# tjysdsg/speech-recognition

Measured on AMD Instinct MI355X. Metric: frame-state loglik/s + utterances/s Viterbi decode, higher is better.
Workload: dtype f64; 1 GPU; configs[1]: 10-digit HMM, 5 states/digit, 8-mix GMM, 39-dim, 10000 utterances/GPU (999364 frames on rank 0), isolated-word decode; states=50, mixtures=8, dim=39, parallelism=utterance-sharded x1, batches_in_flight=2, process_group=single

## Files before the change

include/gmmhmm.h:

```cpp
#ifndef GMMHMM_H
#define GMMHMM_H

#include <stdint.h>

#ifdef __cplusplus
extern "C" {
#endif

typedef enum {
    GH_OK = 0,
    GH_ERR_INVALID = -1,
    GH_ERR_HIP = -2,
    GH_ERR_NOMEM = -3,
    GH_ERR_NODEVICE = -4,
    GH_ERR_SELF_POINTER = -5,
    GH_ERR_UNSUPPORTED = -6,
    GH_ERR_COMM = -7
} gh_status;

typedef enum { GH_F32 = 0, GH_F64 = 1 } gh_dtype;

typedef struct gh_ctx gh_ctx;
typedef struct gh_gmm gh_gmm;
typedef struct gh_batch gh_batch;
// ... 56 lines not shown
                 int64_t* end , int32_t* n_segments , uint8_t* open ,
                 int64_t* frames_done , const int64_t* frame_off , uint8_t* out_is_speech,
                 double* out_level, double* out_background, double* out_energy);
int gh_batch_create_from_pcm_endpointed(gh_ctx* ctx, gh_dtype dtype, int mode, int sample_fmt, int sample_rate,
                                        double frame_size, double frame_stride, double low_freq, double high_freq, int64_t U,
                                        const void* samples, const int64_t* sample_off, const gh_endpoint_params* prm,
                                        int start_boundary, int max_segments, int64_t* start, int64_t* end,
                                        int32_t* n_segments, uint8_t* open, int64_t* utt_frame_off, int64_t* n_utt,
                                        gh_batch** out);

int gh_loglik(gh_ctx* ctx, const gh_gmm* g, gh_batch* b, void* out_host );
int gh_loglik_subset(gh_ctx* ctx, const gh_gmm* g, gh_batch* b, const int32_t* state_lo ,
                     const int32_t* state_hi );
int gh_loglik_sets(gh_ctx* ctx, const gh_gmm* g, gh_batch* b, const int64_t* range_off ,
                   const int32_t* state_lo, const int32_t* state_hi);
void* gh_loglik_dev_ptr(gh_batch* b);
int gh_loglik_fetch(gh_ctx* ctx, const gh_batch* b, void* out_host );
int gh_component_loglik(gh_ctx* ctx, const gh_gmm* g, int state, int64_t N,
                        const double* x_host , double* out_host );
int gh_distance_matrix(gh_ctx* ctx, int64_t N, int K, int D, const double* x_host ,
                       const double* y_host , const double* var_host, int var_rows,
                       double* out_host );

int gh_lattices_create(gh_ctx* ctx, int L,
                       const int64_t* row_off , const int32_t* row_state,
                       const int64_t* arc_off , const int32_t* arc_to,
                       const int32_t* arc_from, const double* arc_cost,
                       const int64_t* start_off , const int32_t* start_rows,
                       const int64_t* end_off , const int32_t* end_rows,
                       gh_lattices** out);
// ... 134 lines not shown
```

speech-recognition_amd/csrc/gh_ctx.hip:

```cpp
#include "gh_internal.h"
#include "gh_host.h"

static thread_local std::string g_err;

void gh_set_error(const char* fmt, ...) {
    char buf[1024];
    va_list ap;
    va_start(ap, fmt);
    vsnprintf(buf, sizeof buf, fmt, ap);
    va_end(ap);
    g_err = buf;
}

extern "C" const char* gh_last_error(void) { return g_err.c_str(); }
extern "C" int gh_version(void) { return 1; }

extern "C" int gh_ctx_create(int device, gh_ctx** out) {
    GH_REQUIRE(out, "gh_ctx_create: out is NULL");
    *out = nullptr;
    int n = 0;
    hipError_t e = hipGetDeviceCount(&n);
    if (e != hipSuccess || n <= 0) {
        gh_set_error("gh_ctx_create: no HIP device (%s)", hipGetErrorString(e));
        return GH_ERR_NODEVICE;
// ... 5 lines not shown
    c->scratch = nullptr;
    c->scratch_bytes = 0;
    c->pinned = nullptr;
    c->pinned_bytes = 0;
    c->last_chunks = 0;
    c->compat = 1;
    if (const char* e = getenv("GMMHMM_COMPAT")) c->compat = strstr(e, "underflow") ? 1 : atoi(e);
    if (const char* e = getenv("GMMHMM_LSE")) if (!strcmp(e, "f32exp")) c->compat |= 2;
    hipDeviceProp_t prop;
    GH_HIP(hipGetDeviceProperties(&prop, device));
    c->n_cu = prop.multiProcessorCount;
    GH_HIP(hipStreamCreateWithFlags(&c->stream, hipStreamNonBlocking));
    GH_HIP(hipMalloc((void**)&c->d_flag, sizeof(int)));
    GH_HIP(hipMemset(c->d_flag, 0, sizeof(int)));
    {
        double t[384];
        for (int j = 0; j < 128; ++j) {
            t[j] = (double)exp2l((long double)j / 128.0L);
            const double inv = (double)(1.0L / (0.5L + ((long double)j + 0.5L) / 256.0L));
            t[128 + j] = inv;
            t[256 + j] = (double)(-logl((long double)inv) * (long double)GH_LSE_SCALE64);
        }
        GH_HIP(hipMalloc((void**)&c->d_fp64_tables, sizeof t));
        GH_HIP(hipMemcpy(c->d_fp64_tables, t, sizeof t, hipMemcpyHostToDevice));
    }
    *out = c;
    return GH_OK;
}

extern "C" void gh_ctx_destroy(gh_ctx* c) {
    if (!c) return;
    hipSetDevice(c->device);
    hipStreamSynchronize(c->stream);
    if (c->scratch) hipFree(c->scratch);
    if (c->pinned) hipHostFree(c->pinned);
    if (c->fit_arena) hipFree(c->fit_arena);
    if (c->fit_pin) hipHostFree(c->fit_pin);
// ... 115 lines not shown
```

speech-recognition_amd/csrc/gh_internal.h:

```cpp
#pragma once
#include <hip/hip_runtime.h>
#include <stdint.h>
#include <stdarg.h>
#include <stdio.h>
#include <string>
#include <vector>
#include "../../include/gmmhmm.h"

void gh_set_error(const char* fmt, ...);

#define GH_HIP(call)                                                                     \
    do {                                                                                 \
        hipError_t e_ = (call);                                                          \
        if (e_ != hipSuccess) {                                                          \
            gh_set_error("%s:%d %s -> %s", __FILE__, __LINE__, #call, hipGetErrorString(e_)); \
            return (e_ == hipErrorOutOfMemory) ? GH_ERR_NOMEM : GH_ERR_HIP;              \
        }                                                                                \
    } while (0)

#define GH_REQUIRE(cond, ...)                 \
    do {                                      \
        if (!(cond)) {                        \
            gh_set_error(__VA_ARGS__);        \
            return GH_ERR_INVALID;            \
// ... 21 lines not shown
    int last_fused = 0;
    int last_chunks;
    size_t budget_cache = 0;
    int budget_age = 0;
    void* fit_arena = nullptr;
    size_t fit_arena_bytes = 0;
    void* fit_pin = nullptr;
    void* fit_act = nullptr;
    size_t fit_act_bytes = 0;
};

int gh_scratch(gh_ctx* ctx, size_t bytes, void** out);
size_t gh_scratch_budget(gh_ctx* ctx, bool fresh = false);
int gh_pinned(gh_ctx* ctx, size_t bytes, void** out);

struct gh_gmm {
    gh_ctx* ctx;
    void* d_arena;
    int S, M, D, KP;
    std::vector<double> hA, hB, hC;
    bool host_stale = false;
    double *dA64, *dB64, *dC64;
    float *dA32, *dB32, *dC32;
    float* dCen32;
    double *dMean, *dIvar, *dLogc;
    int* dAnyPos = nullptr;
    int any_pos_host = -1;
    int M_pad, n_tiles;
    double *dApk64, *dCpk64;
    float *dApk32, *dCpk32;
// ... 189 lines not shown
```

speech-recognition_amd/csrc/gh_loglik_mfma.hip:

```cpp
#include "gh_internal.h"
#include "gh_wave.h"

namespace {

typedef double v4d __attribute__((ext_vector_type(4)));
typedef float v4f __attribute__((ext_vector_type(4)));

struct gh_loglik_blk { int64_t n0; int32_t nrows, t0, t1, pad; };

template <typename T> struct Acc;
template <> struct Acc<double> {
    typedef v4d type;
    static __device__ __forceinline__ v4d mfma(double a, double b, v4d c) {
        return __builtin_amdgcn_mfma_f64_16x16x4f64(a, b, c, 0, 0, 0);
    }
};
template <> struct Acc<float> {
    typedef v4f type;
    static __device__ __forceinline__ v4f mfma(float a, float b, v4f c) {
        return __builtin_amdgcn_mfma_f32_16x16x4f32(a, b, c, 0, 0, 0);
    }
};

struct Fp64Tables {
    double exp2[128];
    double inv[128];
    double nlog[128];
};

template <typename T> struct Dom;
template <> struct Dom<double> {
    static constexpr double inv_k = 1.0 / GH_LSE_SCALE64, off = GH_LSE_OFF64, off_test = GH_LSE_OFF64 * 0.1;
};
template <> struct Dom<float> {
    static constexpr float inv_k = (float)(1.0 / GH_LSE_SCALE32), off = GH_LSE_OFF32, off_test = GH_LSE_OFF32 * 0.1f;
};

struct LseK {
    double e3 = 2.6466421444330968834e-08;
    double l4 = -46.166241308446829036, l3 = 61.554988411262438714;
    double l2 = -92.332482616893658071, l1 = 184.66496523378731614;
    __device__ __forceinline__ void pin() {
        asm volatile("" : "+v"(e3), "+v"(l4), "+v"(l3), "+v"(l2), "+v"(l1));
    }
};

__device__ __forceinline__ double logs(double s, const double* __restrict__ tab, const LseK& k) {
    const double* __restrict__ inv = tab + 128;
    const double* __restrict__ nlog = tab + 256;
    const double m = __builtin_amdgcn_frexp_mant(s);
    const int e = __builtin_amdgcn_frexp_exp(s);
    const int j = (__double2hiint(m) >> 13) & 127;
    const double rho = fma(m, inv[j], -1.0);
    double p = fma(rho, 36.932993046757463228, k.l4);
    p = fma(p, rho, k.l3);
    p = fma(p, rho, k.l2);
    p = fma(p, rho, k.l1);
    return fma(p, rho, nlog[j]) + (double)(e << 7);
}
__device__ __forceinline__ float logs(float s, const double*, const LseK&) { return __builtin_amdgcn_logf(s); }

template <int W> __device__ __forceinline__ void swap_rows(unsigned v, unsigned& a, unsigned& b) {
    if (W == 16) {
        auto r = __builtin_amdgcn_permlane16_swap(v, v, false, false);
        a = r[0]; b = r[1];
    } else {
        auto r = __builtin_amdgcn_permlane32_swap(v, v, false, false);
        a = r[0]; b = r[1];
    }
}
template <int W> __device__ __forceinline__ void pair_of(float v, float& a, float& b) {
    unsigned x, y;
    swap_rows<W>(__float_as_uint(v), x, y);
    a = __uint_as_float(x); b = __uint_as_float(y);
}
// ... 11 lines not shown
}
__device__ __forceinline__ void pair_split(double v0, double v1, double& a, double& b) {
    auto lo = __builtin_amdgcn_permlane16_swap((unsigned)__double2loint(v0), (unsigned)__double2loint(v1), false, false);
    auto hi = __builtin_amdgcn_permlane16_swap((unsigned)__double2hiint(v0), (unsigned)__double2hiint(v1), false, false);
    a = __hiloint2double((int)hi[0], (int)lo[0]); b = __hiloint2double((int)hi[1], (int)lo[1]);
}
template <typename T> __device__ __forceinline__ T pair_sum_split(T v0, T v1) { T a, b; pair_split(v0, v1, a, b); return a + b; }
template <typename T> __device__ __forceinline__ T pair_max_split(T v0, T v1) { T a, b; pair_split(v0, v1, a, b); return vmax(a, b); }

template <typename T> __device__ __forceinline__ T nll_of(T mx, T sm, const double* tab, T inf_below, const LseK& k) {
    const T v = (mx + logs(sm, tab, k)) * -Dom<T>::inv_k;
    return (mx < inf_below) ? T(INFINITY) : v;
}

template <typename T, typename V> __device__ __forceinline__ T lane_max(const V& a) { return vmax(vmax(a[0], a[1]), vmax(a[2], a[3])); }
template <typename T, typename V> __device__ __forceinline__ T lane_terms(const V& a, T m, const double* tab, const LseK& k) {
    return (exp2s(a[0] - m, tab, k.e3) + exp2s(a[1] - m, tab, k.e3)) + (exp2s(a[2] - m, tab, k.e3) + exp2s(a[3] - m, tab, k.e3));
}
template <typename T, typename V>
__device__ __forceinline__ void tile_lse(const V& a, int width, T& mx, T& sm, const double* tab, const LseK& k) {
    T m = lane_max<T, V>(a);
    if (width >= 2) m = pair_max<T, 16>(m);
    if (width >= 4) m = pair_max<T, 32>(m);
    T e = lane_terms<T, V>(a, m, tab, k);
    if (width >= 2) e = pair_sum<T, 16>(e);
    if (width >= 4) e = pair_sum<T, 32>(e);
    mx = m;
    sm = e;
}

__device__ __forceinline__ float exp2s_fe(double y) { return __builtin_amdgcn_exp2f((float)y * 0.0078125f); }
template <int W> __device__ __forceinline__ float pair_sum_f(float v) { float a, b; pair_of<W>(v, a, b); return a + b; }
template <typename V>
__device__ __forceinline__ void tile_lse_fe(const V& a, int width, double& mx, float& sm) {
    double m = vmax(vmax(a[0], a[1]), vmax(a[2], a[3]));
    if (width >= 2) m = pair_max<double, 16>(m);
    if (width >= 4) m = pair_max<double, 32>(m);
    float e = (exp2s_fe(a[0] - m) + exp2s_fe(a[1] - m)) + (exp2s_fe(a[2] - m) + exp2s_fe(a[3] - m));
    if (width >= 2) e = pair_sum_f<16>(e);
// ... 1 lines not shown
    mx = m;
    sm = e;
}
__device__ __forceinline__ double nll_of_fe(double mx, float sm, double inf_below) {
    const double v = (mx + (double)(128.0f * __builtin_amdgcn_logf(sm))) * -Dom<double>::inv_k;
    return (mx < inf_below) ? (double)INFINITY : v;
}

template <typename T> using global_ptr = const T __attribute__((address_space(1)))*;
template <typename T> __device__ __forceinline__ global_ptr<T> uniform_ptr(const T* p) {
    uint32_t lo = (uint32_t)reinterpret_cast<uintptr_t>(p), hi = (uint32_t)(reinterpret_cast<uintptr_t>(p) >> 32);
    asm("" : "+s"(lo), "+s"(hi));
    return (global_ptr<T>)reinterpret_cast<const T*>(((uintptr_t)hi << 32) | lo);
}

template <typename T, typename V, int MP, bool FE = false>
__device__ __forceinline__ void tile_epilogue(const V& acc0, const V& acc1, int t, int f, int q, int S, int RS,
                                              int chunk_s0, int tiles_per_state, T* lds, T* dummy,
                                              const double* tab, T (&run_mx)[2], T (&run_sm)[2], T inf_below, const LseK& k) {
    T* orow0 = lds + f * RS - chunk_s0;
    T* orow1 = orow0 + 16 * RS;
    if (MP == 1) {
        const int s = 16 * t + 4 * q;
#pragma unroll
        for (int c = 0; c < 2; ++c) {
            const V& acc = c ? acc1 : acc0;
            T* orow = c ? orow1 : orow0;
#pragma unroll
            for (int r = 0; r < 4; ++r)
                *((s + r < S) ? orow + s + r : dummy) = (acc[r] < inf_below) ? T(INFINITY) : acc[r] * -Dom<T>::inv_k;
        }
    } else if (MP == 2) {
        const int s = 8 * t + 2 * q;
#pragma unroll
        for (int c = 0; c < 2; ++c) {
            const V& acc = c ? acc1 : acc0;
            T* orow = c ? orow1 : orow0;
#pragma unroll
            for (int h = 0; h < 2; ++h) {
                const T x0 = acc[2 * h], x1 = acc[2 * h + 1];
                const T m = vmax(x0, x1);
                const T e = exp2s(x0 - m, tab, k.e3) + exp2s(x1 - m, tab, k.e3);
                *((s + h < S) ? orow + s + h : dummy) = nll_of<T>(m, e, tab, inf_below, k);
            }
        }
#ifdef GH_MF_NOEPI
    } else if (MP <= 16) {
        const int s = (16 / MP) * t + q / (MP / 4);
        *(((q & (MP / 4 - 1)) == 0 && s < S) ? orow0 + s : dummy) = -((acc0[0] + acc0[1]) + (acc0[2] + acc0[3]));
        *(((q & (MP / 4 - 1)) == 0 && s < S) ? orow1 + s : dummy) = -((acc1[0] + acc1[1]) + (acc1[2] + acc1[3]));
#endif
    } else if (FE && MP == 4) {
        if constexpr (FE) {
            double mx; float sm;
            const int s = 4 * t + q;
            tile_lse_fe<V>(acc0, 1, mx, sm);
            *((s < S) ? orow0 + s : dummy) = nll_of_fe(mx, sm, inf_below);
            tile_lse_fe<V>(acc1, 1, mx, sm);
// ... 24 lines not shown
                run_sm[c] = (double)((d > 0.0) ? fmaf(smf, e, rs) : fmaf(rs, e, smf));
                run_mx[c] = (d > 0.0) ? run_mx[c] : mx;
            }
            const bool odd = q & 1;
            const double v = nll_of_fe(odd ? run_mx[1] : run_mx[0], (float)(odd ? run_sm[1] : run_sm[0]), inf_below);
            *((last && q < 2 && s < S) ? (odd ? orow1 : orow0) + s : dummy) = v;
#pragma unroll
            for (int c = 0; c < 2; ++c) {
                run_mx[c] = last ? Dom<T>::off : run_mx[c];
                run_sm[c] = last ? T(0) : run_sm[c];
            }
        }
    } else if (MP == 4) {
        T mx, sm;
        const int s = 4 * t + q;
        tile_lse<T, V>(acc0, 1, mx, sm, tab, k);
        *((s < S) ? orow0 + s : dummy) = nll_of<T>(mx, sm, tab, inf_below, k);
        tile_lse<T, V>(acc1, 1, mx, sm, tab, k);
        *((s < S) ? orow1 + s : dummy) = nll_of<T>(mx, sm, tab, inf_below, k);
    } else if (MP <= 16) {
        constexpr int width = MP / 4;
        T mxs = pair_max_split(lane_max<T, V>(acc0), lane_max<T, V>(acc1));
        if (width >= 4) mxs = pair_max<T, 32>(mxs);
        T mx0, mx1;
        pair_of<16>(mxs, mx0, mx1);
        T sm = pair_sum_split(lane_terms<T, V>(acc0, mx0, tab, k), lane_terms<T, V>(acc1, mx1, tab, k));
        if (width >= 4) sm = pair_sum<T, 32>(sm);
        const bool odd = q & 1;
        const int s = (16 / MP) * t + q / width;
        const T v = nll_of<T>(mxs, sm, tab, inf_below, k);
        *(((q & (width - 1)) < 2 && s < S) ? (odd ? orow1 : orow0) + s : dummy) = v;
    } else {
        const bool last = (t + 1) % tiles_per_state == 0;
        const int s = t / tiles_per_state;
#pragma unroll
        for (int c = 0; c < 2; ++c) {
            T mx, sm;
            tile_lse<T, V>(c ? acc1 : acc0, 4, mx, sm, tab, k);
            const T d = run_mx[c] - mx;
            const T e = exp2s((d > T(0)) ? -d : d, tab, k.e3);
            run_sm[c] = (d > T(0)) ? fma(sm, e, run_sm[c]) : fma(run_sm[c], e, sm);
            run_mx[c] = (d > T(0)) ? run_mx[c] : mx;
        }
        const bool odd = q & 1;
        const T v = nll_of<T>(odd ? run_mx[1] : run_mx[0], odd ? run_sm[1] : run_sm[0], tab, inf_below, k);
        *((last && q < 2 && s < S) ? (odd ? orow1 : orow0) + s : dummy) = v;
#pragma unroll
        for (int c = 0; c < 2; ++c) {
            run_mx[c] = last ? Dom<T>::off : run_mx[c];
            run_sm[c] = last ? T(0) : run_sm[c];
        }
    }
}

#ifndef GH_MF_SGB
#define GH_MF_SGB 0
#endif
template <typename T, int KS, int MP, bool MULTI, bool FE = false>
__global__ __launch_bounds__(64, (sizeof(T) == 4 ? 3 : 1)) void loglik_mfma_kernel(const T* __restrict__ X, int64_t N, int D,
                                                         const T* __restrict__ Apk, const T* __restrict__ Cpk,
                                                         int n_tiles, int S, int M_pad, int chunk_tiles,
                                                         const double* __restrict__ tables, int tab_off,
                                                         T* __restrict__ out, int bpw,
                                                         const gh_loglik_blk* __restrict__ blk_tab, int64_t n_blk,
                                                         const T* __restrict__ cen, T inf_below) {
    typedef typename Acc<T>::type V;
#ifndef GH_MF_RING32
#define GH_MF_RING32 2
#endif
#ifndef GH_MF_RING64
#define GH_MF_RING64 1
#endif
    constexpr int R = KS / (sizeof(T) == 4 ? GH_MF_RING32 : GH_MF_RING64);
    extern __shared__ __attribute__((aligned(16))) unsigned char smem_raw[];
    T* lds = reinterpret_cast<T*>(smem_raw);
    const int lane = threadIdx.x;
    const int f = lane & 15, q = lane >> 4;
    const int64_t n_blocks = (N + 31) / 32;
    int64_t n0 = (int64_t)blockIdx.x * (MULTI ? bpw : 1) * 32;
#ifdef GH_MF_TIMING
    long long tk[5], tw[2];
    tk[0] = clock64(); tw[0] = wall_clock64();
#endif
    int nrows = 0;
    const bool subset = MULTI && blk_tab != nullptr;
    const int64_t kb0 = (int64_t)blockIdx.x * (MULTI ? bpw : 1);
    int t_lo = subset ? blk_tab[kb0].t0 : 0, t_hi = n_tiles, nxt_t0 = 0;
    double* tab = reinterpret_cast<double*>(smem_raw + tab_off);
    if (sizeof(T) == 8 && MP != 1) {
        double tr[6];
#pragma unroll
        for (int it = 0; it < 6; ++it) tr[it] = tables[lane + 64 * it];
#pragma unroll
        for (int it = 0; it < 6; ++it) tab[lane + 64 * it] = tr[it];
    }
    auto stage_frames = [&]() {
        const int nelem = nrows * D;
        const T* src = X + n0 * D;
        T xr[KS];
#pragma unroll
        for (int it = 0; it < KS; ++it) {
            const int i = lane + 64 * it;
            xr[it] = (i < nelem) ? src[i] : T(0);
        }
#pragma unroll
        for (int it = 0; it < KS; ++it) {
            const int i = lane + 64 * it;
            if (i < nelem) lds[i] = xr[it];
        }
// ... 112 lines not shown
#ifdef GH_MF_PRIO
            __builtin_amdgcn_s_setprio(0);
#endif
            staged_n0 = n0;
        }
        chunk_s0 = (MP <= 16) ? t_lo * (16 / (MP <= 16 ? MP : 16)) : t_lo / tiles_per_state;
        if (subset) {
            const int s_end = (MP <= 16) ? t_hi * (16 / (MP <= 16 ? MP : 16)) : t_hi / tiles_per_state;
            subset_cnt = ((s_end < S) ? s_end : S) - chunk_s0;
        }
#ifdef GH_MF_TIMING
        tk[1] = clock64();
        tk[2] = tk[1];
#endif
        auto epi = [&](const V& e0, const V& e1, int t) {
            tile_epilogue<T, V, MP, FE>(e0, e1, t, f, q, S, RS, chunk_s0, tiles_per_state, lds, dummy, tab, run_mx, run_sm, inf_below, lse_k);
#pragma unroll
            for (int i = 0; i < (GH_MF_SGB ? 2 * KS : 0); ++i) {
                __builtin_amdgcn_sched_group_barrier(0x008, 1, 0);
                __builtin_amdgcn_sched_group_barrier(0x002, sizeof(T) == 8 ? 5 : 3, 0);
            }
            if (!subset && (t + 1) % chunk_tiles == 0 && t + 1 < n_tiles) flush();
        };
        V r0, r1;
        const int tb = MULTI ? t_lo : 0, te = MULTI ? t_hi : n_tiles;
        mfma_tile(tb, p0, p1, c_a, c_b);
        if (sizeof(T) == 8) {
            int t = tb + 1;
            for (; t + 1 < te; t += 2) {
                mfma_tile(t, r0, r1, c_b, c_a);
                epi(p0, p1, t - 1);
// ... 23 lines not shown
        tk[3] = clock64();
#endif
        flush();
#ifdef GH_MF_TIMING
        tk[4] = clock64(); tw[1] = wall_clock64();
        if (lane == 0 && S >= 8) {
            T* o = out + n0 * S;
            for (int i = 0; i < 5; ++i) o[i] = (T)(double)(tk[i] - tk[0]);
            o[5] = (T)(double)(tw[0] & 0xffffffffffll); o[6] = (T)(double)(tw[1] - tw[0]);
            o[7] = (T)(double)__builtin_amdgcn_s_getreg((4 << 0) | (0 << 6) | (31 << 11));
        }
#endif
    }
}

static void chunk_shape(const gh_gmm* g, int* chunk_tiles_out, int* SC_out) {
    const int M_pad = g->M_pad, n_tiles = g->n_tiles, S = g->S;
    int chunk_tiles;
    if (M_pad <= 16) {
        const int spt = 16 / M_pad;
        chunk_tiles = (S <= 64) ? n_tiles : std::max(1, 64 / spt);
    } else {
        const int tps = M_pad / 16;
        chunk_tiles = (S <= 64) ? n_tiles : 64 * tps;
    }
    *chunk_tiles_out = chunk_tiles;
    *SC_out = (M_pad <= 16) ? chunk_tiles * (16 / M_pad) : chunk_tiles / (M_pad / 16);
}

static int build_blk_table(const gh_gmm* g, const gh_batch* b, int SC, const int32_t* st_lo, const int32_t* st_hi,
                           const int64_t* rng_off, std::vector<gh_loglik_blk>& tabv, int* max_tiles_out,
                           const uint8_t* include = nullptr) {
    const int M_pad = g->M_pad, S = g->S;
    int max_tiles = 1;
    std::vector<std::pair<int, int>> runs;
    for (int64_t u = 0; u < b->U; ++u) {
        if (include && !include[u]) continue;
        runs.clear();
        const int64_t r0 = rng_off ? rng_off[u] : u, r1 = rng_off ? rng_off[u + 1] : u + 1;
        for (int64_t r = r0; r < r1; ++r) {
            const int lo = st_lo[r], hi = st_hi[r];
            if (lo < 0 || hi > S || lo >= hi) { gh_set_error("gh_loglik_subset: utterance %lld has state range [%d, %d)", (long long)u, lo, hi); return GH_ERR_INVALID; }
// ... 20 lines not shown
                tabv.push_back(gh_loglik_blk{f, (int32_t)std::min<int64_t>(32, b->offsets[u + 1] - f), tr.first, tr.second, 0});
    }
    *max_tiles_out = max_tiles;
    return GH_OK;
}

template <typename T>
int launch_mfma_t(gh_ctx* ctx, const gh_gmm* g, gh_batch* b, const T* Apk, const T* Cpk, const int32_t* st_lo,
                  const int32_t* st_hi, const T* cen, const int64_t* rng_off, const gh_loglik_plan* plan) {
    const int64_t N = b->N;
    if (N == 0) return GH_OK;
    const int KS = g->KP / 2;
    const int M_pad = g->M_pad, n_tiles = g->n_tiles, S = g->S;
    int chunk_tiles, SC;
    chunk_shape(g, &chunk_tiles, &SC);
    size_t lds = ((size_t)32 * std::max(std::min(SC, S), g->D) + 64) * sizeof(T);
    lds = (lds + 15) & ~size_t(15);
    const int tab_off = (int)lds;
    if (sizeof(T) == 8 && M_pad != 1) lds += 384 * sizeof(double);
    const double* tables = ctx->d_fp64_tables;
    const T inf_below = (ctx->compat & 1) ? (T)(-745.1332191019412 * (sizeof(T) == 8 ? GH_LSE_SCALE64 : GH_LSE_SCALE32)) : Dom<T>::off_test;
    gh_loglik_blk* d_blk = nullptr;
    int64_t n_blk = 0;
    int max_tiles = n_tiles;
    if (plan) {
        d_blk = static_cast<gh_loglik_blk*>(plan->d_blk);
        n_blk = plan->n_blk;
        max_tiles = plan->max_tiles;
        if (n_blk == 0) return GH_OK;
    } else if (st_lo) {
        std::vector<gh_loglik_blk> tabv;
        int rc = build_blk_table(g, b, SC, st_lo, st_hi, rng_off, tabv, &max_tiles);
        if (rc) return rc;
        n_blk = (int64_t)tabv.size();
// ... 3 lines not shown
        if (rc) return rc;
        d_blk = static_cast<gh_loglik_blk*>(base);
        GH_HIP(hipMemcpyAsync(d_blk, tabv.data(), tabv.size() * sizeof(gh_loglik_blk), hipMemcpyHostToDevice, ctx->stream));
        GH_HIP(hipStreamSynchronize(ctx->stream));
    }
    const bool subset = plan || st_lo;
    const int64_t n_blocks = subset ? n_blk : (N + 31) / 32;
    const int per_block = std::max(1, max_tiles * KS * 2);
    int bpw = (int)std::max<int64_t>(1, std::min<int64_t>(8, (512 + per_block - 1) / per_block));
    if (const char* e = getenv("GMMHMM_LOGLIK_BPW")) bpw = std::max(1, std::min(16, atoi(e)));
    if (subset) bpw = std::max(bpw, 2);
    const unsigned grid = (unsigned)((n_blocks + bpw - 1) / bpw);
    const T* X = static_cast<const T*>(b->feats);
    T* out = static_cast<T*>(b->nll);
    const bool fe = sizeof(T) == 8 && (ctx->compat & 2) && M_pad >= 4;
#define GH_MF_LAUNCH(ks, mp)                                                                                             \
    do {                                                                                                                 \
        if (fe && sizeof(T) == 8 && mp >= 4) {                                                                           \
            if (bpw > 1)                                                                                                 \
                hipLaunchKernelGGL((loglik_mfma_kernel<T, ks, mp, true, (sizeof(T) == 8 && mp >= 4)>), dim3(grid), dim3(64), lds, ctx->stream, X, N, g->D, \
                                   Apk, Cpk, n_tiles, S, M_pad, chunk_tiles, tables, tab_off, out, bpw, d_blk, n_blk, cen, inf_below); \
            else                                                                                                         \
                hipLaunchKernelGGL((loglik_mfma_kernel<T, ks, mp, false, (sizeof(T) == 8 && mp >= 4)>), dim3(grid), dim3(64), lds, ctx->stream, X, N, g->D, \
                                   Apk, Cpk, n_tiles, S, M_pad, chunk_tiles, tables, tab_off, out, bpw, d_blk, n_blk, cen, inf_below); \
        } else if (bpw > 1)                                                                                                     \
            hipLaunchKernelGGL((loglik_mfma_kernel<T, ks, mp, true>), dim3(grid), dim3(64), lds, ctx->stream, X, N, g->D, \
                               Apk, Cpk, n_tiles, S, M_pad, chunk_tiles, tables, tab_off, out, bpw, d_blk, n_blk, cen, inf_below); \
        else                                                                                                             \
            hipLaunchKernelGGL((loglik_mfma_kernel<T, ks, mp, false>), dim3(grid), dim3(64), lds, ctx->stream, X, N, g->D, \
                               Apk, Cpk, n_tiles, S, M_pad, chunk_tiles, tables, tab_off, out, bpw, d_blk, n_blk, cen, inf_below); \
    } while (0)
#define GH_MF_CASE(ks)                                   \
    case ks:                                             \
        switch (M_pad) {                                 \
            case 1: GH_MF_LAUNCH(ks, 1); break;          \
            case 2: GH_MF_LAUNCH(ks, 2); break;          \
            case 4: GH_MF_LAUNCH(ks, 4); break;          \
            case 8: GH_MF_LAUNCH(ks, 8); break;          \
            case 16: GH_MF_LAUNCH(ks, 16); break;        \
            default: GH_MF_LAUNCH(ks, 32); break;        \
        }                                                \
        break;
    switch (KS) {
        GH_MF_CASE(2)
        GH_MF_CASE(4)
        GH_MF_CASE(8)
        GH_MF_CASE(12)
        GH_MF_CASE(20)
        GH_MF_CASE(24)
        GH_MF_CASE(32)
        default:
            return 1;
    }
#undef GH_MF_CASE
#undef GH_MF_LAUNCH
    GH_HIP(hipGetLastError());
    return GH_OK;
}

}

int gh_launch_loglik_mfma(gh_ctx* ctx, const gh_gmm* g, gh_batch* b, const int32_t* st_lo, const int32_t* st_hi,
                          const int64_t* rng_off, const gh_loglik_plan* plan) {
    if (!g->dApk64) return 1;
    b->nll_serial = g->serial;
    if (b->dtype == GH_F64) return launch_mfma_t<double>(ctx, g, b, g->dApk64, g->dCpk64, st_lo, st_hi, nullptr, rng_off, plan);
    return launch_mfma_t<float>(ctx, g, b, g->dApk32, g->dCpk32, st_lo, st_hi, g->dCen32, rng_off, plan);
}

int gh_loglik_plan_build(gh_ctx* ctx, const gh_gmm* g, const gh_batch* b, const int32_t* st_lo, const int32_t* st_hi,
                         const int64_t* rng_off, gh_loglik_plan* out, const uint8_t* include) {
    out->d_blk = nullptr; out->n_blk = 0; out->max_tiles = 1;
    if (!g->dApk64) return 1;
    const int KS = g->KP / 2;
    if (KS != 2 && KS != 4 && KS != 8 && KS != 12 && KS != 20 && KS != 24 && KS != 32) return 1;
    int chunk_tiles, SC;
    chunk_shape(g, &chunk_tiles, &SC);
    std::vector<gh_loglik_blk> tabv;
    int rc = build_blk_table(g, b, SC, st_lo, st_hi, rng_off, tabv, &out->max_tiles, include);
    if (rc) return rc;
    out->n_blk = (int64_t)tabv.size();
    if (tabv.empty()) return GH_OK;
// ... 10 lines not shown
```

speech-recognition_amd/csrc/gh_model.hip:

```cpp
#include "gh_internal.h"
#include <atomic>
#include "gh_host.h"

uint64_t gh_next_serial() {
    static std::atomic<uint64_t> counter{0};
    return ++counter;
}

extern "C" int gh_gmm_create(gh_ctx* ctx, int S, int M, int D, const double* mean, const double* var,
                             const double* weight, gh_gmm** out) {
    GH_REQUIRE(ctx && out && mean && var && weight, "gh_gmm_create: NULL argument");
    GH_REQUIRE(S > 0 && M > 0 && D > 0, "gh_gmm_create: S=%d M=%d D=%d must be positive", S, M, D);
    *out = nullptr;
    GH_HIP(hipSetDevice(ctx->device));
    const int G = S * M;
    int KP = (D + 3) & ~3;
    for (const int kp : {4, 8, 16, 24, 40, 48, 64})
        if (KP <= kp) { KP = kp; break; }
    gh_gmm* g = new gh_gmm();
    g->ctx = ctx;
    g->d_arena = nullptr;
    g->S = S; g->M = M; g->D = D; g->KP = KP;
    g->hA.assign((size_t)G * KP, 0.0);
    g->hB.assign((size_t)G * KP, 0.0);
    g->hC.assign(G, 0.0);
    std::vector<double> ivar((size_t)G * D), logc(G);
    const double log2pi = std::log(2.0 * M_PI);
    for (int i = 0; i < G; ++i) {
        double sum_logv = 0, sum_m2 = 0;
        for (int d = 0; d < D; ++d) {
            const double v = var[(size_t)i * D + d], mu = mean[(size_t)i * D + d];
            if (v == 0) {
                delete g;
// ... 21 lines not shown
        }
        cen32[d] = cnt ? (float)(double)(acc / cnt) : 0.f;
        if (!std::isfinite(cen32[d])) cen32[d] = 0.f;
    }
    std::vector<double> hB32((size_t)G * KP, 0.0), hC32(G, 0.0);
    for (int i = 0; i < G; ++i) {
        double sum_m2 = 0;
        for (int d = 0; d < D; ++d) {
            const double iv = ivar[(size_t)i * D + d], mu = mean[(size_t)i * D + d] - (double)cen32[d];
            hB32[(size_t)i * KP + d] = mu * iv;
            sum_m2 += mu * mu * iv;
        }
        hC32[i] = logc[i] - 0.5 * sum_m2;
    }
    std::vector<float> fA(g->hA.begin(), g->hA.end()), fB(hB32.begin(), hB32.end()), fC(hC32.begin(), hC32.end());
    int M_pad = 1;
    if (M <= 16) { while (M_pad < M) M_pad <<= 1; } else { M_pad = (M + 15) & ~15; }
    const int n_tiles = (S * M_pad + 15) / 16, KS = KP / 2;
    g->M_pad = M_pad;
    g->n_tiles = n_tiles;
    g->dApk64 = nullptr; g->dCpk64 = nullptr; g->dApk32 = nullptr; g->dCpk32 = nullptr; g->dCen32 = nullptr;
    std::vector<double> apk64((size_t)(n_tiles + 2) * KS * 64, 0.0), cpk64((size_t)(n_tiles + 2) * 16, GH_LSE_OFF64);
    std::vector<float> apk32(apk64.size(), 0.f), cpk32(cpk64.size(), GH_LSE_OFF32);
    for (int t = 0; t < n_tiles; ++t)
        for (int j = 0; j < 16; ++j) {
            const int gp = t * 16 + j, s = gp / M_pad, m = gp % M_pad;
            if (s >= S || m >= M) continue;
            const int go = s * M + m;
            const double c = g->hC[go], c32 = hC32[go];
            cpk64[gp] = (c == -INFINITY) ? GH_LSE_OFF64 : std::max(c * GH_LSE_SCALE64, GH_LSE_OFF64);
            cpk32[gp] = (c32 == -INFINITY) ? GH_LSE_OFF32 : (float)std::max(c32 * GH_LSE_SCALE32, (double)GH_LSE_OFF32);
            const int row64 = (j >> 2) + 4 * (j & 3), row32 = j;
            for (int ks = 0; ks < KS; ++ks)
// ... 601 lines not shown
```

speech-recognition_amd/sr/recognition/_hip.py:

```python
import ctypes as C
import os
import threading

import numpy as np

_HERE = os.path.dirname(os.path.abspath(__file__))
LIB_PATH = os.environ.get("GMMHMM_LIB") or os.path.normpath(
    os.path.join(_HERE, "..", "..", "lib", "libgmmhmm.so"))

GH_F32, GH_F64 = 0, 1
GH_ERR_SELF_POINTER = -5
GH_ERR_UNSUPPORTED = -6
GH_ERR_COMM = -7

_c_i32p = C.POINTER(C.c_int32)
_c_i64p = C.POINTER(C.c_int64)
_c_f64p = C.POINTER(C.c_double)
_c_u8p = C.POINTER(C.c_uint8)


class EndpointParams(C.Structure):
    _fields_ = [("width", C.c_int32), ("stride", C.c_int32), ("speech_frames", C.c_int32), ("silence_frames", C.c_int32),
                ("forget", C.c_double), ("adjustment", C.c_double), ("onset", C.c_double), ("offset", C.c_double)]

# ... 37 lines not shown
    "gh_mfcc": (C.c_int, [C.c_void_p, C.c_int, C.c_int, C.c_double, C.c_double, C.c_double, C.c_double, C.c_int64,
                          C.c_void_p, _c_i64p, _c_i64p, _c_f64p, _c_f64p]),
    "gh_batch_create_from_pcm": (C.c_int, [C.c_void_p, C.c_int, C.c_int, C.c_int, C.c_int, C.c_double, C.c_double,
                                           C.c_double, C.c_double, C.c_int64, C.c_void_p, _c_i64p, _c_i64p,
                                           C.POINTER(C.c_void_p)]),
    "gh_endpoint_frames": (C.c_int64, [C.c_int64, C.c_int, C.c_int]),
    "gh_endpoints": (C.c_int, [C.c_void_p, C.c_int64, C.c_void_p, _c_i64p, C.POINTER(EndpointParams), C.c_int, _c_i64p, _c_i64p,
                               _c_i32p, _c_u8p, _c_i64p, _c_i64p, _c_u8p, _c_f64p, _c_f64p, _c_f64p]),
    "gh_batch_create_from_pcm_endpointed": (C.c_int, [C.c_void_p, C.c_int, C.c_int, C.c_int, C.c_int, C.c_double, C.c_double,
                                                      C.c_double, C.c_double, C.c_int64, C.c_void_p, _c_i64p,
                                                      C.POINTER(EndpointParams), C.c_int, C.c_int, _c_i64p, _c_i64p, _c_i32p,
                                                      _c_u8p, _c_i64p, _c_i64p, C.POINTER(C.c_void_p)]),
    "gh_loglik": (C.c_int, [C.c_void_p, C.c_void_p, C.c_void_p, C.c_void_p]),
    "gh_loglik_sets": (C.c_int, [C.c_void_p, C.c_void_p, C.c_void_p, _c_i64p, _c_i32p, _c_i32p]),
    "gh_loglik_subset": (C.c_int, [C.c_void_p, C.c_void_p, C.c_void_p, _c_i32p, _c_i32p]),
    "gh_loglik_dev_ptr": (C.c_void_p, [C.c_void_p]),
    "gh_loglik_fetch": (C.c_int, [C.c_void_p, C.c_void_p, C.c_void_p]),
    "gh_component_loglik": (C.c_int, [C.c_void_p, C.c_void_p, C.c_int, C.c_int64, _c_f64p, _c_f64p]),
    "gh_distance_matrix": (C.c_int, [C.c_void_p, C.c_int64, C.c_int, C.c_int, _c_f64p, _c_f64p, _c_f64p,
                                     C.c_int, _c_f64p]),
    "gh_lattices_create": (C.c_int, [C.c_void_p, C.c_int, _c_i64p, _c_i32p, _c_i64p, _c_i32p, _c_i32p,
                                     _c_f64p, _c_i64p, _c_i32p, _c_i64p, _c_i32p, C.POINTER(C.c_void_p)]),
    "gh_lattices_create_transcripts": (C.c_int, [C.c_void_p, C.c_int, C.c_int, _c_f64p, _c_i32p, C.c_int64, _c_i64p, _c_i32p,
                                                 C.POINTER(C.c_void_p)]),
    "gh_lattices_destroy": (None, [C.c_void_p]),
    "gh_lattices_set_beam": (C.c_int, [C.c_void_p, C.c_int]),
    "gh_lattices_forms": (C.c_int, [C.c_void_p]),
    "gh_viterbi": (C.c_int, [C.c_void_p, C.c_void_p, C.c_void_p, _c_i32p, _c_f64p, _c_i32p, _c_i32p, _c_i64p,
                             _c_i32p, _c_f64p, _c_i64p]),
    "gh_viterbi_fused": (C.c_int, [C.c_void_p, C.c_void_p, C.c_void_p, C.c_void_p, C.c_int, _c_f64p, _c_i32p, _c_i32p, _c_i64p,
# ... 1191 lines not shown
```

Measured before the change: 41.39 billion frame-state loglik/s.

## Use 256-entry LDS exp2 table with byte-index addressing in f64 loglik epilogue

Adds a 256-entry duplicated exp2 table placed at LDS offset zero, so the exp2 lookup index can be formed with a single SDWA shift of the low byte of the rounded exponent, with no separate mask or base-add. It also adds a 'full' variant that drops the s<S bounds checks when S divides evenly into tiles, and uses a readfirstlane scalar offset for the f64 output store. The plan function keeps the larger table only when occupancy (workgroups per CU within the LDS budget) does not drop. The cost is more LDS per block and extra kernel instantiations, plus inline asm that relies on the table sitting at LDS address 0.

```diff
diff --git a/include/gmmhmm.h b/include/gmmhmm.h
--- a/include/gmmhmm.h
+++ b/include/gmmhmm.h
@@ -94,6 +94,7 @@
                      const int32_t* state_hi );
 int gh_loglik_sets(gh_ctx* ctx, const gh_gmm* g, gh_batch* b, const int64_t* range_off ,
                    const int32_t* state_lo, const int32_t* state_hi);
+int gh_loglik_lds_plan(int S, int M, int D, int dtype, int blocks_per_wave, int64_t* out );
 void* gh_loglik_dev_ptr(gh_batch* b);
 int gh_loglik_fetch(gh_ctx* ctx, const gh_batch* b, void* out_host );
 int gh_component_loglik(gh_ctx* ctx, const gh_gmm* g, int state, int64_t N,
diff --git a/speech-recognition_amd/csrc/gh_ctx.hip b/speech-recognition_amd/csrc/gh_ctx.hip
--- a/speech-recognition_amd/csrc/gh_ctx.hip
+++ b/speech-recognition_amd/csrc/gh_ctx.hip
@@ -43,13 +43,15 @@
     GH_HIP(hipMalloc((void**)&c->d_flag, sizeof(int)));
     GH_HIP(hipMemset(c->d_flag, 0, sizeof(int)));
     {
-        double t[384];
+        double t[384 + 512];
         for (int j = 0; j < 128; ++j) {
             t[j] = (double)exp2l((long double)j / 128.0L);
             const double inv = (double)(1.0L / (0.5L + ((long double)j + 0.5L) / 256.0L));
             t[128 + j] = inv;
             t[256 + j] = (double)(-logl((long double)inv) * (long double)GH_LSE_SCALE64);
         }
+        for (int j = 0; j < 256; ++j) t[384 + j] = t[j & 127];
+        for (int j = 0; j < 256; ++j) t[384 + 256 + j] = t[128 + j];
         GH_HIP(hipMalloc((void**)&c->d_fp64_tables, sizeof t));
         GH_HIP(hipMemcpy(c->d_fp64_tables, t, sizeof t, hipMemcpyHostToDevice));
     }
diff --git a/speech-recognition_amd/csrc/gh_internal.h b/speech-recognition_amd/csrc/gh_internal.h
--- a/speech-recognition_amd/csrc/gh_internal.h
+++ b/speech-recognition_amd/csrc/gh_internal.h
@@ -59,6 +59,14 @@
 size_t gh_scratch_budget(gh_ctx* ctx, bool fresh = false);
 int gh_pinned(gh_ctx* ctx, size_t bytes, void** out);
 
+static inline void gh_gmm_pad_shape(int S, int M, int D, int* KP_out, int* M_pad_out, int* n_tiles_out) {
+    int KP = (D + 3) & ~3;
+    for (const int kp : {4, 8, 16, 24, 40, 48, 64})
+        if (KP <= kp) { KP = kp; break; }
+    int M_pad = 1;
+    if (M <= 16) { while (M_pad < M) M_pad <<= 1; } else { M_pad = (M + 15) & ~15; }
+    *KP_out = KP; *M_pad_out = M_pad; *n_tiles_out = (S * M_pad + 15) / 16;
+}
 struct gh_gmm {
     gh_ctx* ctx;
     void* d_arena;
diff --git a/speech-recognition_amd/csrc/gh_loglik_mfma.hip b/speech-recognition_amd/csrc/gh_loglik_mfma.hip
--- a/speech-recognition_amd/csrc/gh_loglik_mfma.hip
+++ b/speech-recognition_amd/csrc/gh_loglik_mfma.hip
@@ -27,6 +27,13 @@
     double inv[128];
     double nlog[128];
 };
+struct Fp64TablesX2 {
+    double exp2[256];
+    double inv[128];
+    double nlog[128];
+};
+constexpr int GH_MF_X2_BYTES = (int)sizeof(Fp64TablesX2);
+constexpr int GH_MF_X2_SRC = (int)(sizeof(Fp64Tables) / 8);
 
 template <typename T> struct Dom;
 template <> struct Dom<double> {
@@ -56,9 +63,28 @@
     p = fma(p, rho, k.l3);
     p = fma(p, rho, k.l2);
     p = fma(p, rho, k.l1);
-    return fma(p, rho, nlog[j]) + (double)(e << 7);
+    return fma((double)e, 128.0, fma(p, rho, nlog[j]));
 }
 __device__ __forceinline__ float logs(float s, const double*, const LseK&) { return __builtin_amdgcn_logf(s); }
+
+__device__ __forceinline__ double exp2s_x2(double y, double c3) {
+    const double n = __builtin_rint(y);
+    const double r = y - n;
+    const int ni = (int)n;
+    unsigned off;
+    asm("v_lshlrev_b32_sdwa %0, 3, %1 dst_sel:DWORD dst_unused:UNUSED_PAD src0_sel:DWORD src1_sel:BYTE_0" : "=v"(off) : "v"(ni));
+    const double t = *reinterpret_cast<const __attribute__((address_space(3))) double*>((uintptr_t)off);
+    double p = fma(r, 3.583032305400251285e-11, c3);
+    p = fma(p, r, 1.4662262387640424337e-05);
+    p = fma(p, r, 5.4152123481245727298e-03);
+    p = p * r;
+    return __builtin_ldexp(fma(t, p, t), ni >> 7);
+}
+template <int IX> __device__ __forceinline__ double ex2(double y, const double* tab, double c3) {
+    if constexpr (IX != 0) return exp2s_x2(y, c3);
+    else return exp2s(y, tab, c3);
+}
+template <int IX> __device__ __forceinline__ float ex2(float y, const double* tab, double c3) { return exp2s(y, tab, c3); }
 
 template <int W> __device__ __forceinline__ void swap_rows(unsigned v, unsigned& a, unsigned& b) {
     if (W == 16) {
@@ -100,15 +126,15 @@
 }
 
 template <typename T, typename V> __device__ __forceinline__ T lane_max(const V& a) { return vmax(vmax(a[0], a[1]), vmax(a[2], a[3])); }
-template <typename T, typename V> __device__ __forceinline__ T lane_terms(const V& a, T m, const double* tab, const LseK& k) {
-    return (exp2s(a[0] - m, tab, k.e3) + exp2s(a[1] - m, tab, k.e3)) + (exp2s(a[2] - m, tab, k.e3) + exp2s(a[3] - m, tab, k.e3));
-}
-template <typename T, typename V>
+template <typename T, typename V, int IX> __device__ __forceinline__ T lane_terms(const V& a, T m, const double* tab, const LseK& k) {
+    return (ex2<IX>(a[0] - m, tab, k.e3) + ex2<IX>(a[1] - m, tab, k.e3)) + (ex2<IX>(a[2] - m, tab, k.e3) + ex2<IX>(a[3] - m, tab, k.e3));
+}
+template <typename T, typename V, int IX>
 __device__ __forceinline__ void tile_lse(const V& a, int width, T& mx, T& sm, const double* tab, const LseK& k) {
     T m = lane_max<T, V>(a);
     if (width >= 2) m = pair_max<T, 16>(m);
     if (width >= 4) m = pair_max<T, 32>(m);
-    T e = lane_terms<T, V>(a, m, tab, k);
+    T e = lane_terms<T, V, IX>(a, m, tab, k);
     if (width >= 2) e = pair_sum<T, 16>(e);
     if (width >= 4) e = pair_sum<T, 32>(e);
     mx = m;
@@ -140,12 +166,13 @@
     return (global_ptr<T>)reinterpret_cast<const T*>(((uintptr_t)hi << 32) | lo);
 }
 
-template <typename T, typename V, int MP, bool FE = false>
+template <typename T, typename V, int MP, bool FE = false, int IX = 0>
 __device__ __forceinline__ void tile_epilogue(const V& acc0, const V& acc1, int t, int f, int q, int S, int RS,
                                               int chunk_s0, int tiles_per_state, T* lds, T* dummy,
                                               const double* tab, T (&run_mx)[2], T (&run_sm)[2], T inf_below, const LseK& k) {
     T* orow0 = lds + f * RS - chunk_s0;
     T* orow1 = orow0 + 16 * RS;
+    constexpr bool FULL = IX == 2;
     if (MP == 1) {
         const int s = 16 * t + 4 * q;
 #pragma unroll
@@ -166,8 +193,8 @@
             for (int h = 0; h < 2; ++h) {
                 const T x0 = acc[2 * h], x1 = acc[2 * h + 1];
                 const T m = vmax(x0, x1);
-                const T e = exp2s(x0 - m, tab, k.e3) + exp2s(x1 - m, tab, k.e3);
-                *((s + h < S) ? orow + s + h : dummy) = nll_of<T>(m, e, tab, inf_below, k);
+                const T e = ex2<IX>(x0 - m, tab, k.e3) + ex2<IX>(x1 - m, tab, k.e3);
+                *((FULL || s + h < S) ? orow + s + h : dummy) = nll_of<T>(m, e, tab, inf_below, k);
             }
         }
 #ifdef GH_MF_NOEPI
@@ -222,31 +249,37 @@
     } else if (MP == 4) {
         T mx, sm;
         const int s = 4 * t + q;
-        tile_lse<T, V>(acc0, 1, mx, sm, tab, k);
-        *((s < S) ? orow0 + s : dummy) = nll_of<T>(mx, sm, tab, inf_below, k);
-        tile_lse<T, V>(acc1, 1, mx, sm, tab, k);
-        *((s < S) ? orow1 + s : dummy) = nll_of<T>(mx, sm, tab, inf_below, k);
+        tile_lse<T, V, IX>(acc0, 1, mx, sm, tab, k);
+        *((FULL || s < S) ? orow0 + s : dummy) = nll_of<T>(mx, sm, tab, inf_below, k);
+        tile_lse<T, V, IX>(acc1, 1, mx, sm, tab, k);
+        *((FULL || s < S) ? orow1 + s : dummy) = nll_of<T>(mx, sm, tab, inf_below, k);
     } else if (MP <= 16) {
         constexpr int width = MP / 4;
         T mxs = pair_max_split(lane_max<T, V>(acc0), lane_max<T, V>(acc1));
         if (width >= 4) mxs = pair_max<T, 32>(mxs);
         T mx0, mx1;
         pair_of<16>(mxs, mx0, mx1);
-        T sm = pair_sum_split(lane_terms<T, V>(acc0, mx0, tab, k), lane_terms<T, V>(acc1, mx1, tab, k));
+        T sm = pair_sum_split(lane_terms<T, V, IX>(acc0, mx0, tab, k), lane_terms<T, V, IX>(acc1, mx1, tab, k));
         if (width >= 4) sm = pair_sum<T, 32>(sm);
         const bool odd = q & 1;
         const int s = (16 / MP) * t + q / width;
         const T v = nll_of<T>(mxs, sm, tab, inf_below, k);
-        *(((q & (width - 1)) < 2 && s < S) ? (odd ? orow1 : orow0) + s : dummy) = v;
+        if constexpr (sizeof(T) == 8) {
+            T* own = lds + (f + (odd ? 16 : 0)) * RS + q / width;
+            const int so = __builtin_amdgcn_readfirstlane((16 / MP) * t - chunk_s0);
+            *(((q & (width - 1)) < 2 && (FULL || s < S)) ? own + so : dummy) = v;
+        } else {
+            *(((q & (width - 1)) < 2 && s < S) ? (odd ? orow1 : orow0) + s : dummy) = v;
+        }
     } else {
         const bool last = (t + 1) % tiles_per_state == 0;
         const int s = t / tiles_per_state;
 #pragma unroll
         for (int c = 0; c < 2; ++c) {
             T mx, sm;
-            tile_lse<T, V>(c ? acc1 : acc0, 4, mx, sm, tab, k);
+            tile_lse<T, V, IX>(c ? acc1 : acc0, 4, mx, sm, tab, k);
             const T d = run_mx[c] - mx;
-            const T e = exp2s((d > T(0)) ? -d : d, tab, k.e3);
+            const T e = ex2<IX>((d > T(0)) ? -d : d, tab, k.e3);
             run_sm[c] = (d > T(0)) ? fma(sm, e, run_sm[c]) : fma(run_sm[c], e, sm);
             run_mx[c] = (d > T(0)) ? run_mx[c] : mx;
         }
@@ -264,7 +297,7 @@
 #ifndef GH_MF_SGB
 #define GH_MF_SGB 0
 #endif
-template <typename T, int KS, int MP, bool MULTI, bool FE = false>
+template <typename T, int KS, int MP, bool MULTI, bool FE = false, int IX = 0>
 __global__ __launch_bounds__(64, (sizeof(T) == 4 ? 3 : 1)) void loglik_mfma_kernel(const T* __restrict__ X, int64_t N, int D,
                                                          const T* __restrict__ Apk, const T* __restrict__ Cpk,
                                                          int n_tiles, int S, int M_pad, int chunk_tiles,
@@ -281,7 +314,7 @@
 #endif
     constexpr int R = KS / (sizeof(T) == 4 ? GH_MF_RING32 : GH_MF_RING64);
     extern __shared__ __attribute__((aligned(16))) unsigned char smem_raw[];
-    T* lds = reinterpret_cast<T*>(smem_raw);
+    T* lds = reinterpret_cast<T*>(smem_raw + (IX ? GH_MF_X2_BYTES : 0));
     const int lane = threadIdx.x;
     const int f = lane & 15, q = lane >> 4;
     const int64_t n_blocks = (N + 31) / 32;
@@ -294,13 +327,16 @@
     const bool subset = MULTI && blk_tab != nullptr;
     const int64_t kb0 = (int64_t)blockIdx.x * (MULTI ? bpw : 1);
     int t_lo = subset ? blk_tab[kb0].t0 : 0, t_hi = n_tiles, nxt_t0 = 0;
-    double* tab = reinterpret_cast<double*>(smem_raw + tab_off);
+    double* tab = reinterpret_cast<double*>(smem_raw + (IX ? 128 * 8 : tab_off));
     if (sizeof(T) == 8 && MP != 1) {
-        double tr[6];
-#pragma unroll
-        for (int it = 0; it < 6; ++it) tr[it] = tables[lane + 64 * it];
-#pragma unroll
-        for (int it = 0; it < 6; ++it) tab[lane + 64 * it] = tr[it];
+        constexpr int TN = (IX ? sizeof(Fp64TablesX2) : sizeof(Fp64Tables)) / (64 * 8);
+        const double* tsrc = tables + (IX ? GH_MF_X2_SRC : 0);
+        double* tdst = IX ? reinterpret_cast<double*>(smem_raw) : tab;
+        double tr[TN];
+#pragma unroll
+        for (int it = 0; it < TN; ++it) tr[it] = tsrc[lane + 64 * it];
+#pragma unroll
+        for (int it = 0; it < TN; ++it) tdst[lane + 64 * it] = tr[it];
     }
     auto stage_frames = [&]() {
         const int nelem = nrows * D;
@@ -443,7 +479,7 @@
         tk[2] = tk[1];
 #endif
         auto epi = [&](const V& e0, const V& e1, int t) {
-            tile_epilogue<T, V, MP, FE>(e0, e1, t, f, q, S, RS, chunk_s0, tiles_per_state, lds, dummy, tab, run_mx, run_sm, inf_below, lse_k);
+            tile_epilogue<T, V, MP, FE, IX>(e0, e1, t, f, q, S, RS, chunk_s0, tiles_per_state, lds, dummy, tab, run_mx, run_sm, inf_below, lse_k);
 #pragma unroll
             for (int i = 0; i < (GH_MF_SGB ? 2 * KS : 0); ++i) {
                 __builtin_amdgcn_sched_group_barrier(0x008, 1, 0);
@@ -497,8 +533,7 @@
     }
 }
 
-static void chunk_shape(const gh_gmm* g, int* chunk_tiles_out, int* SC_out) {
-    const int M_pad = g->M_pad, n_tiles = g->n_tiles, S = g->S;
+static void chunk_shape(int M_pad, int n_tiles, int S, int* chunk_tiles_out, int* SC_out) {
     int chunk_tiles;
     if (M_pad <= 16) {
         const int spt = 16 / M_pad;
@@ -509,6 +544,33 @@
     }
     *chunk_tiles_out = chunk_tiles;
     *SC_out = (M_pad <= 16) ? chunk_tiles * (16 / M_pad) : chunk_tiles / (M_pad / 16);
+}
+static void chunk_shape(const gh_gmm* g, int* chunk_tiles_out, int* SC_out) { chunk_shape(g->M_pad, g->n_tiles, g->S, chunk_tiles_out, SC_out); }
+
+struct mf_lds_plan {
+    size_t tile;
+    size_t lds128, lds;
+    int wg128, wg;
+    int ix;
+};
+constexpr size_t GH_CU_LDS = 160 * 1024;
+static mf_lds_plan mf_plan(int S, int D, int M_pad, int n_tiles, int KS, size_t esz, bool multi, bool fe, bool force128) {
+    int chunk_tiles, SC;
+    chunk_shape(M_pad, n_tiles, S, &chunk_tiles, &SC);
+    mf_lds_plan p;
+    p.tile = (((size_t)32 * std::max(std::min(SC, S), D) + 64) * esz + 15) & ~size_t(15);
+    const bool tables = esz == 8 && M_pad != 1;
+    const int reg_wg = (esz == 8 && KS >= 20) ? 8 : 32;
+    p.lds128 = p.tile + (tables ? sizeof(Fp64Tables) : 0);
+    p.wg128 = (int)std::min<size_t>(GH_CU_LDS / p.lds128, reg_wg);
+    const size_t lds256 = p.tile + sizeof(Fp64TablesX2);
+    const int wg256 = (int)std::min<size_t>(GH_CU_LDS / lds256, reg_wg);
+    p.ix = 0; p.lds = p.lds128; p.wg = p.wg128;
+    if (tables && !fe && !force128 && wg256 >= p.wg128) {
+        const bool full = M_pad <= 16 && S % (16 / M_pad) == 0;
+        p.ix = (full && !multi) ? 2 : 1; p.lds = lds256; p.wg = wg256;
+    }
+    return p;
 }
 
 static int build_blk_table(const gh_gmm* g, const gh_batch* b, int SC, const int32_t* st_lo, const int32_t* st_hi,
@@ -559,10 +621,6 @@
     const int M_pad = g->M_pad, n_tiles = g->n_tiles, S = g->S;
     int chunk_tiles, SC;
     chunk_shape(g, &chunk_tiles, &SC);
-    size_t lds = ((size_t)32 * std::max(std::min(SC, S), g->D) + 64) * sizeof(T);
-    lds = (lds + 15) & ~size_t(15);
-    const int tab_off = (int)lds;
-    if (sizeof(T) == 8 && M_pad != 1) lds += 384 * sizeof(double);
     const double* tables = ctx->d_fp64_tables;
     const T inf_below = (ctx->compat & 1) ? (T)(-745.1332191019412 * (sizeof(T) == 8 ? GH_LSE_SCALE64 : GH_LSE_SCALE32)) : Dom<T>::off_test;
     gh_loglik_blk* d_blk = nullptr;
@@ -596,21 +654,36 @@
     const T* X = static_cast<const T*>(b->feats);
     T* out = static_cast<T*>(b->nll);
     const bool fe = sizeof(T) == 8 && (ctx->compat & 2) && M_pad >= 4;
+    const char* tab_env = getenv("GMMHMM_LOGLIK_TAB");
+    const mf_lds_plan lp = mf_plan(S, g->D, M_pad, n_tiles, KS, sizeof(T), bpw > 1, fe, tab_env && atoi(tab_env) == 128);
+    const size_t lds = lp.lds;
+    const int tab_off = (int)lp.tile, ix = lp.ix;
+    if (const char* e = getenv("GMMHMM_HOST_TRACE"))
+        if (atoi(e) && sizeof(T) == 8 && M_pad != 1 && !fe) fprintf(stderr, "loglik_tab=%d full=%d\n", ix ? 256 : 128, ix == 2);
+#define GH_MF_ARGS dim3(grid), dim3(64), lds, ctx->stream, X, N, g->D, Apk, Cpk, n_tiles, S, M_pad, chunk_tiles, tables, tab_off, out, bpw, d_blk, n_blk, cen, inf_below
 #define GH_MF_LAUNCH(ks, mp)                                                                                             \
     do {                                                                                                                 \
         if (fe && sizeof(T) == 8 && mp >= 4) {                                                                           \
             if (bpw > 1)                                                                                                 \
-                hipLaunchKernelGGL((loglik_mfma_kernel<T, ks, mp, true, (sizeof(T) == 8 && mp >= 4)>), dim3(grid), dim3(64), lds, ctx->stream, X, N, g->D, \
-                                   Apk, Cpk, n_tiles, S, M_pad, chunk_tiles, tables, tab_off, out, bpw, d_blk, n_blk, cen, inf_below); \
+                hipLaunchKernelGGL((loglik_mfma_kernel<T, ks, mp, true, (sizeof(T) == 8 && mp >= 4)>), GH_MF_ARGS);      \
             else                                                                                                         \
-                hipLaunchKernelGGL((loglik_mfma_kernel<T, ks, mp, false, (sizeof(T) == 8 && mp >= 4)>), dim3(grid), dim3(64), lds, ctx->stream, X, N, g->D, \
-                                   Apk, Cpk, n_tiles, S, M_pad, chunk_tiles, tables, tab_off, out, bpw, d_blk, n_blk, cen, inf_below); \
-        } else if (bpw > 1)                                                                                                     \
-            hipLaunchKernelGGL((loglik_mfma_kernel<T, ks, mp, true>), dim3(grid), dim3(64), lds, ctx->stream, X, N, g->D, \
-                               Apk, Cpk, n_tiles, S, M_pad, chunk_tiles, tables, tab_off, out, bpw, d_blk, n_blk, cen, inf_below); \
+                hipLaunchKernelGGL((loglik_mfma_kernel<T, ks, mp, false, (sizeof(T) == 8 && mp >= 4)>), GH_MF_ARGS);     \
+        } else if (ix != 0) {                                                                                            \
+            if constexpr (sizeof(T) == 8 && mp >= 2) {                                                                   \
+                if (bpw > 1)                                                                                             \
+                    hipLaunchKernelGGL((loglik_mfma_kernel<T, ks, mp, true, false, 1>), GH_MF_ARGS);                     \
+                else if (ix == 2)                                                                                        \
+                    hipLaunchKernelGGL((loglik_mfma_kernel<T, ks, mp, false, false, (mp <= 16 ? 2 : 1)>), GH_MF_ARGS);   \
+                else                                                                                                     \
+                    hipLaunchKernelGGL((loglik_mfma_kernel<T, ks, mp, false, false, 1>), GH_MF_ARGS);                    \
+            } else {                                                                                                     \
+                gh_set_error("gh_loglik: index form %d without an instantiation", ix);                                   \
+                return GH_ERR_INVALID;                                                                                   \
+            }                                                                                                            \
+        } else if (bpw > 1)                                                                                              \
+            hipLaunchKernelGGL((loglik_mfma_kernel<T, ks, mp, true>), GH_MF_ARGS);                                       \
         else                                                                                                             \
-            hipLaunchKernelGGL((loglik_mfma_kernel<T, ks, mp, false>), dim3(grid), dim3(64), lds, ctx->stream, X, N, g->D, \
-                               Apk, Cpk, n_tiles, S, M_pad, chunk_tiles, tables, tab_off, out, bpw, d_blk, n_blk, cen, inf_below); \
+            hipLaunchKernelGGL((loglik_mfma_kernel<T, ks, mp, false>), GH_MF_ARGS);                                      \
     } while (0)
 #define GH_MF_CASE(ks)                                   \
     case ks:                                             \
@@ -636,6 +709,7 @@
     }
 #undef GH_MF_CASE
 #undef GH_MF_LAUNCH
+#undef GH_MF_ARGS
     GH_HIP(hipGetLastError());
     return GH_OK;
 }
@@ -648,6 +722,16 @@
     b->nll_serial = g->serial;
     if (b->dtype == GH_F64) return launch_mfma_t<double>(ctx, g, b, g->dApk64, g->dCpk64, st_lo, st_hi, nullptr, rng_off, plan);
     return launch_mfma_t<float>(ctx, g, b, g->dApk32, g->dCpk32, st_lo, st_hi, g->dCen32, rng_off, plan);
+}
+
+extern "C" int gh_loglik_lds_plan(int S, int M, int D, int dtype, int blocks_per_wave, int64_t* out) {
+    GH_REQUIRE(out && S > 0 && M > 0 && D > 0 && D <= 64, "gh_loglik_lds_plan: bad argument");
+    int KP, M_pad, n_tiles;
+    gh_gmm_pad_shape(S, M, D, &KP, &M_pad, &n_tiles);
+    const mf_lds_plan p = mf_plan(S, D, M_pad, n_tiles, KP / 2, dtype == GH_F64 ? 8 : 4, blocks_per_wave > 1, false, false);
+    out[0] = (int64_t)p.lds128; out[1] = p.wg128; out[2] = (int64_t)p.lds; out[3] = p.wg;
+    out[4] = p.ix ? 256 : 128; out[5] = p.ix == 2;
+    return GH_OK;
 }
 
 int gh_loglik_plan_build(gh_ctx* ctx, const gh_gmm* g, const gh_batch* b, const int32_t* st_lo, const int32_t* st_hi,
diff --git a/speech-recognition_amd/csrc/gh_model.hip b/speech-recognition_amd/csrc/gh_model.hip
--- a/speech-recognition_amd/csrc/gh_model.hip
+++ b/speech-recognition_amd/csrc/gh_model.hip
@@ -14,9 +14,8 @@
     *out = nullptr;
     GH_HIP(hipSetDevice(ctx->device));
     const int G = S * M;
-    int KP = (D + 3) & ~3;
-    for (const int kp : {4, 8, 16, 24, 40, 48, 64})
-        if (KP <= kp) { KP = kp; break; }
+    int KP, M_pad, n_tiles;
+    gh_gmm_pad_shape(S, M, D, &KP, &M_pad, &n_tiles);
     gh_gmm* g = new gh_gmm();
     g->ctx = ctx;
     g->d_arena = nullptr;
@@ -68,9 +67,7 @@
         hC32[i] = logc[i] - 0.5 * sum_m2;
     }
     std::vector<float> fA(g->hA.begin(), g->hA.end()), fB(hB32.begin(), hB32.end()), fC(hC32.begin(), hC32.end());
-    int M_pad = 1;
-    if (M <= 16) { while (M_pad < M) M_pad <<= 1; } else { M_pad = (M + 15) & ~15; }
-    const int n_tiles = (S * M_pad + 15) / 16, KS = KP / 2;
+    const int KS = KP / 2;
     g->M_pad = M_pad;
     g->n_tiles = n_tiles;
     g->dApk64 = nullptr; g->dCpk64 = nullptr; g->dApk32 = nullptr; g->dCpk32 = nullptr; g->dCen32 = nullptr;
diff --git a/speech-recognition_amd/sr/recognition/_hip.py b/speech-recognition_amd/sr/recognition/_hip.py
--- a/speech-recognition_amd/sr/recognition/_hip.py
+++ b/speech-recognition_amd/sr/recognition/_hip.py
@@ -75,6 +75,7 @@
     "gh_loglik": (C.c_int, [C.c_void_p, C.c_void_p, C.c_void_p, C.c_void_p]),
     "gh_loglik_sets": (C.c_int, [C.c_void_p, C.c_void_p, C.c_void_p, _c_i64p, _c_i32p, _c_i32p]),
     "gh_loglik_subset": (C.c_int, [C.c_void_p, C.c_void_p, C.c_void_p, _c_i32p, _c_i32p]),
+    "gh_loglik_lds_plan": (C.c_int, [C.c_int, C.c_int, C.c_int, C.c_int, C.c_int, _c_i64p]),
     "gh_loglik_dev_ptr": (C.c_void_p, [C.c_void_p]),
     "gh_loglik_fetch": (C.c_int, [C.c_void_p, C.c_void_p, C.c_void_p]),
     "gh_component_loglik": (C.c_int, [C.c_void_p, C.c_void_p, C.c_int, C.c_int64, _c_f64p, _c_f64p]),
```

New measurement: 41.11 billion frame-state loglik/s. Within noise of the previous version (-0.7%).
